# peterhpark/neuroclear

Measured on AMD Instinct MI355X. Metric: voxels/sec, higher is better.
Workload: dtype f32

## Files before the change

### include/nc_hip.h

```cpp
#ifndef NC_HIP_H
#define NC_HIP_H

#include <stddef.h>
#include <stdint.h>

#ifdef __cplusplus
extern "C" {
#endif

#define NC_OK 0
#define NC_ERR_SHAPE (-1)
#define NC_ERR_WS (-2)
#define NC_ERR_HIP (-3)
#define NC_ERR_ARG (-4)

const char* nc_last_error(void);
int nc_version(void);
int nc_conv_fwd_path(int C, int K, int kd, int kh, int kw, int stride, int pad);
int nc_conv_wgrad_path(int C, int K, int kd, int kh, int kw, int stride, int pad);
void nc_prof_begin(double min_flop);
int nc_prof_end(int max, int* cls, double* flop, float* ms);
int nc_prof_end2(int max, int* cls, double* flop, float* ms, double* abytes);
void nc_set_force_direct(int on);
void nc_sconv_set_cfg(int cfg);
// ... 128 lines not shown
int nc_assemble_scatter_add(const float* cube, float* acc, int P0, int P1, int P2, int roi, int overlap, int border,
                            int index, void* stream);
int nc_assemble_finalize(const float* acc, void* out, int out_is_u16, int P0, int P1, int P2, int L0, int L1, int L2,
                         int roi, int overlap, void* stream);
int nc_assemble_finalize_slab(const float* acc_slab, void* out, int out_is_u16, int P0, int P1, int P2, int L0, int L1, int L2, int roi,
                              int overlap, int z0, int nz, int za, void* stream);

int nc_assemble_merge(const float* acc, float* merged, int L0, int L1, int L2, int roi, int overlap, void* stream);
int nc_radix_hist(const float* x, long n, int pass, unsigned prefix, unsigned* hist4096, void* stream);
int nc_assemble_rescale_finalize(const float* merged, void* out, int out_is_u16, int L0, int L1, int L2, int roi,
                                 int overlap, float lo, float hi, float range, void* stream);

size_t nc_match_histograms_ws_bytes(long n);
int nc_match_histograms(const float* source, const float* tmpl, float* out, long n, void* ws, size_t ws_bytes,
                        void* stream);

int nc_spectral_norm_fwd(const float* w_orig, float* u, float* v, float* w_out, float* sigma, float* scratch_k, int K, int M,
                         int power_iteration, float eps, void* stream);
int nc_spectral_norm_bwd(const float* g, const float* w_sn, const float* u, const float* v, const float* sigma, float* dw_orig, int K,
                         int M, void* stream);

size_t nc_patchgan_param_floats(int n_layers, int ndf, int nd);
size_t nc_patchgan_saved_floats(int B, int D, int H, int W, int n_layers, int ndf, int nd);
size_t nc_patchgan_ws_bytes(int B, int D, int H, int W, int n_layers, int ndf, int nd);
int nc_patchgan_out_shape(int B, int D, int H, int W, int n_layers, int ndf, int nd, int* oD, int* oH, int* oW);
int nc_patchgan_fwd(const float* params, const float* x, float* y, float* saved, int B, int D, int H, int W,
                    int n_layers, int ndf, int nd, void* ws, size_t ws_bytes, void* stream);
int nc_patchgan_bwd(const float* params, const float* x, const float* saved, const float* dy, float* dx, float* dparams,
                    int B, int D, int H, int W, int n_layers, int ndf, int nd, void* ws, size_t ws_bytes, void* stream);
int nc_patchgan_fwd_part(const float* params, const float* x, float* y, float* saved, int Btot, int b0, int B, int D, int H,
                         int W, int n_layers, int ndf, int nd, void* ws, size_t ws_bytes, void* stream);
int nc_patchgan_bwd_part(const float* params, const float* x, const float* saved, const float* dy, float* dx, int Btot, int b0,
                         int B, int D, int H, int W, int n_layers, int ndf, int nd, void* ws, size_t ws_bytes, void* stream);
size_t nc_patchgan_gp_saved_floats(int B, int D, int H, int W, int n_layers, int ndf, int nd);
size_t nc_patchgan_gp_ws_bytes(int B, int D, int H, int W, int n_layers, int ndf, int nd);
int nc_patchgan_gp_fwd(const float* params, const float* x, float* g, float* pen, float* saved, int B, int D, int H, int W, int n_layers,
                       int ndf, int nd, float constant, float lambda_gp, void* ws, size_t ws_bytes, void* stream);
int nc_patchgan_gp_bwd(const float* params, const float* x, const float* saved, const float* g, const float* dpen, float* dparams, float* dx,
                       int B, int D, int H, int W, int n_layers, int ndf, int nd, float constant, float lambda_gp, void* ws, size_t ws_bytes,
                       void* stream);

size_t nc_unet_deconv_fwd_ws_bytes(int N, int S0, int S1, int S2);
int nc_unet_deconv_fwd(const float* params, const float* x, float* y, int N, int S0, int S1, int S2, void* ws,
                       size_t ws_bytes, void* stream);


size_t nc_unet_deconv_param_floats(void);
size_t nc_unet_deconv_saved_floats(int N, int S0, int S1, int S2);
size_t nc_unet_deconv_train_ws_bytes(int N, int S0, int S1, int S2);
int nc_unet_deconv_train_fwd(const float* params, const float* x, float* y, float* saved, int N, int S0, int S1, int S2,
                             void* ws, size_t ws_bytes, void* stream, unsigned* kept);
int nc_unet_deconv_bwd(const float* params, const float* x, const float* y, const float* saved, const float* dy, float* dx,
                       float* dparams, int N, int S0, int S1, int S2, void* ws, size_t ws_bytes, void* stream, unsigned kept);
void nc_set_unet_lean(int on);
int nc_get_unet_lean(void);
void nc_set_unet_wprep(int on);
int nc_get_unet_wprep(void);
int nc_set_in_bwd_fold(int on);
int nc_get_in_bwd_fold(void);
int nc_in_bwd_launches(int which, int reset);
int nc_set_stream_passes(int on);
int nc_get_stream_passes(void);
int nc_unet_wprep_layout(int N, int S0, int S1, int S2, int block, int form, size_t* pack_off, size_t* pack_bytes, size_t* cell_off,
                         size_t* bound_off);
int nc_s3x_pack_h2_debug(const float* w, int C, int K, int form, const unsigned* cell_a, const unsigned* cell_b, void* wp, unsigned* wcell,
                         void* stream);
// ... 138 lines not shown
```

### neuroclear_amd/csrc/common.hpp

```cpp
#pragma once
#include <hip/hip_runtime.h>

#include <cstdarg>
#include <cstdio>

#include "../../include/nc_hip.h"
#include "switches.hpp"

namespace nc {

void set_error(const char* fmt, ...);

inline int check_launch(const char* what) {
  hipError_t e = hipGetLastError();
  if (e != hipSuccess) {
    set_error("%s: %s", what, hipGetErrorString(e));
    return NC_ERR_HIP;
  }
  return NC_OK;
}

inline long cdiv(long a, long b) { return (a + b - 1) / b; }

int raise_dyn_lds(const void* kernel, int bytes, const char* who);
// ... 49 lines not shown

int conv_fwd_direct(const float* x, const float* w, const float* b, float* y, const ConvDims& d, hipStream_t s);
int conv_dgrad_direct(const float* dy, const float* w, float* dx, const ConvDims& d, hipStream_t s);
int conv_wgrad_direct(const float* x, const float* dy, float* dw, const ConvDims& d, hipStream_t s);
int bias_grad(const float* dy, float* db, int N, int K, long S, void* ws, size_t wsb, hipStream_t s);
static constexpr size_t kBiasGradWsBytes = 64 * 1024 * sizeof(double);

bool mfma_fwd_supported(const ConvDims& d);
bool c1k3_fwd_supported(const ConvDims& d);
int conv_fwd_c1k3(const float* x, const float* w, const float* bias, float* y, const ConvDims& d, hipStream_t s, float* stats_part = nullptr);
size_t c1k3_stats_bytes(const ConvDims& d);
int c1k3_stats_finalize(const float* stats_part, const float* bias, const ConvDims& d, float eps, float* mean, float* rstd, hipStream_t s);
bool mfma_dgrad_supported(const ConvDims& d);
bool mfma_wgrad_supported(const ConvDims& d);
size_t mfma_ws_bytes(const ConvDims& d);
size_t mfma_fwd_ws_bytes(const ConvDims& d);
int conv_fwd_mfma(const float* x, const float* w, const float* b, float* y, const ConvDims& d, void* ws, size_t wsb,
                  hipStream_t s);
int conv_dgrad_mfma(const float* dy, const float* w, float* dx, const ConvDims& d, void* ws, size_t wsb,
                    hipStream_t s);
int conv_wgrad_mfma(const float* x, const float* dy, float* dw, const ConvDims& d, void* ws, size_t wsb,
                    hipStream_t s);

bool gemm_fwd_supported(const ConvDims& d);
bool gemm_dgrad_supported(const ConvDims& d);
bool gemm_wgrad_supported(const ConvDims& d);
size_t gemm_ws_bytes(const ConvDims& d);
int conv_fwd_gemm(const float* x, const float* w, const float* b, float* y, const ConvDims& d, void* ws, size_t wsb,
                  hipStream_t s);
int conv_dgrad_gemm(const float* dy, const float* w, float* dx, const ConvDims& d, void* ws, size_t wsb,
                    hipStream_t s);
int conv_wgrad_gemm(const float* x, const float* dy, float* dw, const ConvDims& d, void* ws, size_t wsb,
                    hipStream_t s);

bool sconv_fwd_supported(const ConvDims& d);
bool sconv_dgrad_supported(const ConvDims& d);
size_t sconv_ws_bytes(const ConvDims& d);
bool p2d_fwd_supported(const ConvDims& d);
bool p2d_dgrad_supported(const ConvDims& d);
size_t p2d_ws_bytes(const ConvDims& d);
int conv_fwd_p2d(const float* x, const float* w, const float* bias, float* y, const ConvDims& d, void* ws, size_t wsb, hipStream_t s);
int conv_dgrad_p2d(const float* dy, const float* w, float* dx, const ConvDims& d, void* ws, size_t wsb, hipStream_t s);
bool p2d_wgrad_supported(const ConvDims& d);
size_t p2d_wgrad_ws_bytes(const ConvDims& d);
int conv_wgrad_p2d(const float* x, const float* dy, float* dw, const ConvDims& d, void* ws, size_t wsb, hipStream_t s);
int conv_fwd_sconv(const float* x, const float* w, const float* bias, float* y, const ConvDims& d, void* ws, size_t wsb, hipStream_t s);
int conv_dgrad_sconv(const float* dy, const float* w, float* dx, const ConvDims& d, void* ws, size_t wsb, hipStream_t s);
int conv2d_k3_num_cfgs();
bool conv2d_k3_fwd_supported(const ConvDims& d);
bool conv2d_k3_dgrad_supported(const ConvDims& d);
size_t conv2d_k3_ws_bytes(const ConvDims& d);
int conv_fwd_k3(const float* x, const float* w, const float* bias, float* y, const ConvDims& d, void* ws, size_t wsb, hipStream_t s);
int conv_dgrad_k3(const float* dy, const float* w, float* dx, const ConvDims& d, void* ws, size_t wsb, hipStream_t s);
bool conv2d_k3_reflect_ok(const ConvDims& d);
int conv_fwd_k3_reflect(const float* x, const float* w, const float* bias, float* y, const ConvDims& d, void* ws, size_t wsb, hipStream_t s);
int conv_dgrad_k3_reflect_ext(const float* dy, const float* w, float* dxe, const ConvDims& d, void* ws, size_t wsb, hipStream_t s);
int reflect_pad_fwd(const float* x, float* y, long NC, int H, int W, int p, hipStream_t s);
int reflect_pad_bwd(const float* g, float* dx, long NC, int H, int W, int p, hipStream_t s);
bool sconv_wgrad_supported(const ConvDims& d);
size_t sconv_wgrad_ws_bytes(const ConvDims& d);
int conv_wgrad_sconv(const float* x, const float* dy, float* dw, const ConvDims& d, void* ws, size_t wsb, hipStream_t s);

bool pg1_supported(const ConvDims& d);
size_t pg1_ws_bytes(const ConvDims& d);
int conv_fwd_pg1(const float* x, const float* w, const float* bias, float* y, const ConvDims& d, float slope, hipStream_t s);
int conv_wgrad_pg1(const float* x, const float* g, const float* act, float slope, float* dw, float* db, const ConvDims& d,
// ... 239 lines not shown
```

### neuroclear_amd/csrc/misc.hip

```cpp
#include "common.hpp"

namespace nc {

__device__ __forceinline__ void plane_dims(int D, int H, int W, int axis, int& A, int& B) {
  A = axis == 0 ? H : D;
  B = axis == 2 ? H : W;
}
__device__ __forceinline__ long vol_index(int D, int H, int W, int axis, int a, int b, int s) {
  if (axis == 0) return ((long)s * H + a) * W + b;
  if (axis == 1) return ((long)a * H + s) * W + b;
  return ((long)a * H + b) * W + s;
}

__global__ void k_slice_bwd(const float* __restrict__ dout, float* __restrict__ dvol, int NC, int D, int H, int W,
                            int axis, int index) {
  int A, B;
  plane_dims(D, H, W, axis, A, B);
  const long S = (long)D * H * W, total = (long)NC * S;
  for (long i = (long)blockIdx.x * blockDim.x + threadIdx.x; i < total; i += (long)gridDim.x * blockDim.x) {
    const long nc = i / S, r = i % S;
    const int x = (int)(r % W), y = (int)((r / W) % H), z = (int)(r / ((long)W * H));
    const int s = axis == 0 ? z : axis == 1 ? y : x;
    const int a = axis == 0 ? y : z;
    const int b = axis == 2 ? y : x;
// ... 96 lines not shown
}
__global__ void k_l1_bwd(const float* __restrict__ a, const float* __restrict__ b, long n,
                         const float* __restrict__ gscale, float* __restrict__ da) {
  const float g = gscale[0] / (float)n;
  for (long i = (long)blockIdx.x * blockDim.x + threadIdx.x; i < n; i += (long)gridDim.x * blockDim.x) {
    const float d = a[i] - b[i];
    da[i] = d > 0.f ? g : d < 0.f ? -g : 0.f;
  }
}

__global__ void k_adam(float* __restrict__ p, const float* __restrict__ g, float* __restrict__ m,
                       float* __restrict__ v, long n, float b1, float b2, float eps, float step_size,
                       float bc2_sqrt) {
  for (long i = (long)blockIdx.x * blockDim.x + threadIdx.x; i < n; i += (long)gridDim.x * blockDim.x) {
    const float gi = g[i];
    const float wl = 1.f - b1;
    const float mi = wl < 0.5f ? m[i] + wl * (gi - m[i]) : gi - (gi - m[i]) * (1.f - wl);
    const float vi = v[i] * b2 + gi * gi * (1.f - b2);
    m[i] = mi;
    v[i] = vi;
    const float denom = sqrtf(vi) / bc2_sqrt + eps;
    p[i] = p[i] - step_size * (mi / denom);
  }
}

static unsigned flat_grid(long n) {
  long b = cdiv(n, 256);
  if (b > 8192) b = 8192;
  if (b < 1) b = 1;
  return (unsigned)b;
}
static constexpr int kLossBlocks = 256;

}

using namespace nc;

extern "C" {

static int vol_check(const char* what, int NC, int D, int H, int W, int axis) {
  if (NC < 1 || D < 1 || H < 1 || W < 1 || axis < 0 || axis > 2) {
    set_error("%s: bad shape/axis", what);
    return NC_ERR_SHAPE;
  }
  return NC_OK;
}
static int axis_len(int D, int H, int W, int axis) { return axis == 0 ? D : axis == 1 ? H : W; }

int nc_slice_fwd(const float* vol, float* out, int NC, int D, int H, int W, int axis, int index, void* stream) {
  if (!vol || !out) { set_error("slice_fwd: null pointer"); return NC_ERR_ARG; }
  if (int e = vol_check("slice_fwd", NC, D, H, W, axis)) return e;
  if (index < 0 || index >= axis_len(D, H, W, axis)) { set_error("slice_fwd: index out of range"); return NC_ERR_SHAPE; }
  hipLaunchKernelGGL(k_mip_fwd, dim3(flat_grid((long)NC * D * H * W / axis_len(D, H, W, axis))), dim3(256), 0,
                     (hipStream_t)stream, vol, out, (int32_t*)nullptr, NC, D, H, W, axis, index, 1);
  return check_launch("slice_fwd");
}
int nc_slice_bwd(const float* dout, float* dvol, int NC, int D, int H, int W, int axis, int index, void* stream) {
  if (!dout || !dvol) { set_error("slice_bwd: null pointer"); return NC_ERR_ARG; }
  if (int e = vol_check("slice_bwd", NC, D, H, W, axis)) return e;
  if (index < 0 || index >= axis_len(D, H, W, axis)) { set_error("slice_bwd: index out of range"); return NC_ERR_SHAPE; }
  hipLaunchKernelGGL(k_slice_bwd, dim3(flat_grid((long)NC * D * H * W)), dim3(256), 0, (hipStream_t)stream, dout, dvol,
                     NC, D, H, W, axis, index);
  return check_launch("slice_bwd");
}
int nc_mip_fwd(const float* vol, float* out, int32_t* arg, int NC, int D, int H, int W, int axis, int start, int depth,
               void* stream) {
// ... 92 lines not shown
```

### neuroclear_amd/csrc/nets.hip

```cpp
#include "common.hpp"
#include "patchgan_plan.hpp"

using namespace nc;

namespace {

size_t align256(size_t b) { return (b + 255) & ~(size_t)255; }

}

#define NC_TRY(expr) do { int e_ = (expr); if (e_) return e_; } while (0)

extern "C" {

size_t nc_patchgan_param_floats(int n_layers, int ndf, int nd) {
  PgPlan P;
  return pg_plan(P, 1, nd == 3 ? 64 : 1, 64, 64, n_layers, ndf, nd) ? P.params : 0;
}

size_t nc_patchgan_saved_floats(int B, int D, int H, int W, int n_layers, int ndf, int nd) {
  PgPlan P;
  return pg_plan(P, B, D, H, W, n_layers, ndf, nd) ? P.saved : 0;
}

// ... 107 lines not shown
        NC_TRY(nc_instnorm_act_bwd_dbias(gin, praw, mean, rstd, 0.2f, graw, dparams + pl.b_off, B, pl.K, S, iws, P.in_ws,
                                         stream));
        have_db = true;
      } else {
        NC_TRY(nc_instnorm_act_bwd(gin, praw, mean, rstd, 0.2f, graw, B * pl.K, S, iws, P.in_ws, stream));
      }
    } else if (i == 1 && P.fused0) {
      graw = gin;
    } else {
      NC_TRY(nc_leaky_relu_bwd(gin, praw, 0.2f, graw, (long)B * pl.K * S, stream));
    }
    g = graw;
  }
  return NC_OK;
}

int nc_patchgan_bwd(const float* params, const float* x, const float* saved, const float* dy, float* dx, float* dparams,
                    int B, int D, int H, int W, int n_layers, int ndf, int nd, void* ws, size_t ws_bytes, void* stream) {
  if (!params || !x || !saved || !dy) { set_error("patchgan_bwd: null pointer"); return NC_ERR_ARG; }
  PgPlan P;
  if (!pg_plan(P, B, D, H, W, n_layers, ndf, nd)) { set_error("patchgan_bwd: bad shape"); return NC_ERR_SHAPE; }
  if (!ws || ws_bytes < nc_patchgan_ws_bytes(B, D, H, W, n_layers, ndf, nd)) { set_error("patchgan_bwd: workspace too small"); return NC_ERR_WS; }
  return pg_bwd(P, params, x, saved, dy, dx, dparams, B, 0, B, nd, ws, stream);
}

int nc_patchgan_bwd_part(const float* params, const float* x, const float* saved, const float* dy, float* dx, int Btot, int b0,
                         int B, int D, int H, int W, int n_layers, int ndf, int nd, void* ws, size_t ws_bytes, void* stream) {
  if (!params || !x || !saved || !dy || !dx) { set_error("patchgan_bwd_part: null pointer"); return NC_ERR_ARG; }
  PgPlan P;
  if (B < 1 || b0 < 0 || b0 + B > Btot || !pg_plan(P, Btot, D, H, W, n_layers, ndf, nd)) { set_error("patchgan_bwd_part: bad shape"); return NC_ERR_SHAPE; }
  if (!ws || ws_bytes < nc_patchgan_ws_bytes(Btot, D, H, W, n_layers, ndf, nd)) { set_error("patchgan_bwd_part: workspace too small"); return NC_ERR_WS; }
  return pg_bwd(P, params, x, saved, dy, dx, nullptr, Btot, b0, B, nd, ws, stream);
}
}
```

### neuroclear_amd/models/axial_to_lateral_gan_apollo_model.py

```python
import itertools
import os

import numpy as np
import torch

from .. import ops
from . import networks
from .base_model import BaseModel


class FlatAdam(torch.optim.Optimizer):

    def __init__(self, params, lr, betas, eps=1e-8, overlap_all_reduce=False):
        params = list(params)
        super().__init__(params, dict(lr=lr, betas=betas, eps=eps))
        self.params = params
        dev = params[0].device
        n = sum(p.numel() for p in params)
        self.flat = torch.empty(n, dtype=torch.float32, device=dev)
        self.grad = torch.zeros(n, dtype=torch.float32, device=dev)
        self.exp_avg = torch.zeros(n, dtype=torch.float32, device=dev)
        self.exp_avg_sq = torch.zeros(n, dtype=torch.float32, device=dev)
        off = 0
        for p in params:
# ... 77 lines not shown
                else:
                    dist.all_reduce(self.grad[b['lo']:b['hi']])
                b['work'], b['seen'] = None, 0
        else:
            dist.all_reduce(self.grad)
        self.grad.div_(ws)

    @torch.no_grad()
    def step(self, closure=None):
        self._collect()
        self.state_step += 1
        g = self.param_groups[0]
        ops.adam_step(self.flat, self.grad, self.exp_avg, self.exp_avg_sq, g['lr'], g['betas'][0], g['betas'][1],
                      g['eps'], self.state_step)
        ops.bump_param_generation(self.flat)


class AxialToLateralGANApolloModel(BaseModel):
    @staticmethod
    def modify_commandline_options(parser, is_train=True):
        parser.set_defaults(no_dropout=True)
        if is_train:
            parser.add_argument('--lambda_A', type=float, default=10.0, help='weight for cycle loss (A -> B -> A)')
            parser.add_argument('--gan_mode', type=str, default='vanilla', help='[vanilla| lsgan | wgangp]')
            parser.add_argument('--lambda_plane', type=int, nargs='+', default=[1, 1, 1])
            parser.add_argument('--randomize_projection_depth', action='store_true')
            parser.add_argument('--projection_depth', type=int, default=10)
            parser.add_argument('--min_projection_depth', type=int, default=2)
        parser.add_argument('--netG_B', type=str, default='deep_linear_gen')
        return parser

    _d_streams_on = os.environ.get('NC_D_STREAMS', '1') != '0'
    _d_on_main = os.environ.get('NC_D_MAIN', '1') != '0'
    _d_nstreams = int(os.environ.get('NC_D_NSTREAMS', '4'))

    def __init__(self, opt):
        BaseModel.__init__(self, opt)
        self._d_streams = []
        self._fwd_done = None
        self.loss_names = ['D_A_lateral', 'D_A_axial', 'G_A', 'G_A_lateral', 'G_A_axial', 'cycle',
                           'D_B_lateral', 'D_B_axial', 'G_B', 'G_B_lateral', 'G_B_axial']
        self.gan_mode = opt.gan_mode
        self.gen_dimension, self.dis_dimension = 3, 2
        self.randomize_projection_depth = opt.randomize_projection_depth
        if not self.randomize_projection_depth:
            self.projection_depth_custom = opt.projection_depth
        else:
            self.max_projection_depth = opt.projection_depth
            self.min_projection_depth = opt.min_projection_depth
        self.visual_names = ['real', 'fake', 'rec'] * 2
        tot = float(opt.lambda_plane[0] + opt.lambda_plane[1] + opt.lambda_plane[2])
        self.lambda_plane_target, self.lambda_slice, self.lambda_proj = [f / tot for f in opt.lambda_plane]
        self.lateral_axis, self.axial_1_axis, self.axial_2_axis = 0, 1, 2
        self.model_names = ['G_A', 'G_B', 'D_A_lateral', 'D_A_axial', 'D_B_lateral', 'D_B_axial'] if self.isTrain \
            else ['G_A', 'G_B']
        G = networks.define_G
        self.netG_A = G(opt.input_nc, opt.output_nc, opt.ngf, opt.netG, opt.norm, not opt.no_dropout, opt.init_type,
                        opt.init_gain, self.gpu_ids, dimension=self.gen_dimension)
        self.netG_B = G(opt.output_nc, opt.input_nc, opt.ngf, opt.netG_B, opt.norm, not opt.no_dropout, opt.init_type,
                        opt.init_gain, self.gpu_ids, dimension=self.gen_dimension)
        if self.isTrain:
            def D(nc):
                return networks.define_D(nc, opt.ndf, opt.netD, opt.n_layers_D, opt.norm, opt.init_type,
                                         opt.init_gain, False, self.gpu_ids, dimension=self.dis_dimension)
            self.netD_A_axial = D(opt.output_nc)
            self.netD_A_lateral = D(opt.output_nc)
# ... 19 lines not shown
        self.cube_shape = self.real.shape
        self.num_slice = self.cube_shape[-3]
        if not self.randomize_projection_depth:
            self.projection_depth = self.projection_depth_custom
        else:
            self.projection_depth = np.random.randint(max(2, self.min_projection_depth),
                                                      self.max_projection_depth + 1)

    _early_DA = os.environ.get('NC_D_EARLY', '0') != '0'

    def forward(self):
        self.fake = self.netG_A(self.real)
        self._fake_done = None
        if self.real.is_cuda and self._d_streams_on and self._early_DA and self.isTrain:
            self._fake_done = torch.cuda.Event()
            self._fake_done.record()
        self.rec = self.netG_B(self.fake)

    def _slice(self, input, slice_axis):
        return ops.volume_slice(input, slice_axis, np.random.randint(input.shape[-1]))

    def _proj(self, input, slice_axis):
        start = np.random.randint(0, input.shape[-1] - self.projection_depth)
        return ops.volume_mip(input, slice_axis, start, self.projection_depth)

    @staticmethod
    def _D(netD, planes):
        if getattr(netD, 'one_plane_per_call', False):
            return [netD(pl) for pl in planes]
        pred = netD(planes[0] if len(planes) == 1 else torch.cat(planes, 0))
        n = planes[0].shape[0]
        return [pred[i * n:(i + 1) * n] for i in range(len(planes))]

    def _D_many(self, jobs, loss_fn, after=None, backward=False):
        def run(i, net, planes_fn):
            res = loss_fn(i, self._D(net, planes_fn()))
            if backward:
                tot = res if torch.is_tensor(res) else sum(res[1:], res[0])
                tot.backward()
            return res
        if not self._d_streams_on or not self.real.is_cuda:
            return [run(i, net, fn) for i, (net, fn) in enumerate(jobs)]
        main = torch.cuda.current_stream()
        on_main = self._d_on_main and len(jobs) > 3 and not backward
        nside = len(jobs) - 1 if on_main else len(jobs)
        ns = min(nside, self._d_nstreams)
        while len(self._d_streams) < ns:
            self._d_streams.append(torch.cuda.Stream(device=self.device))
        out = []
        for i, (net, fn) in enumerate(jobs[:nside]):
            st = self._d_streams[i % ns]
            ev = after[i] if isinstance(after, (list, tuple)) else after
            if ev is not None:
                st.wait_event(ev)
            else:
                st.wait_stream(main)
            with torch.cuda.stream(st):
                out.append(run(i, net, fn))
        if on_main:
            out.append(run(nside, *jobs[nside]))
        for i in range(ns):
            main.wait_stream(self._d_streams[i])
        return out

    def iter_f(self, input, function, slice_axis):
        return function(self._slice(input, slice_axis))

    def proj_f(self, input, function, slice_axis):
        return function(self._proj(input, slice_axis))
# ... 25 lines not shown
        self.loss_D_A_axial_1 = self._d_loss(p[0], p[1])
        self.loss_D_A_axial_2 = self._d_loss(p[2], p[3])
        (self.loss_D_A_axial_1 + self.loss_D_A_axial_2).backward()
        self.loss_D_A_axial = (self.loss_D_A_axial_1 + self.loss_D_A_axial_2) * 0.5

    def backward_D_B_lateral(self):
        self.loss_D_B_lateral = self.backward_D_slice(self.netD_B_lateral, self.real, self.rec, self.lateral_axis,
                                                      self.lateral_axis)

    def backward_D_B_axial(self):
        rd = self.rec.detach()
        planes = [self._slice(self.real, self.axial_1_axis), self._slice(rd, self.axial_1_axis),
                  self._slice(self.real, self.axial_2_axis), self._slice(rd, self.axial_2_axis)]
        p = self._D(self.netD_B_axial, planes)
        self.loss_D_B_axial_1 = self._d_loss(p[0], p[1])
        self.loss_D_B_axial_2 = self._d_loss(p[2], p[3])
        (self.loss_D_B_axial_1 + self.loss_D_B_axial_2).backward()
        self.loss_D_B_axial = (self.loss_D_B_axial_1 + self.loss_D_B_axial_2) * 0.5

    def backward_G(self):
        lambda_A = self.opt.lambda_A
        g = self.criterionGAN
        f, r = self.fake, self.rec
        la, a1, a2 = self.lateral_axis, self.axial_1_axis, self.axial_2_axis
        jobs = [(self.netD_A_lateral, lambda: [self._proj(f, la)]),
                (self.netD_A_axial, lambda: [self._proj(f, a1), self._proj(f, a2)]),
                (self.netD_B_lateral, lambda: [self._slice(r, la)]),
                (self.netD_B_axial, lambda: [self._slice(r, a1), self._slice(r, a2)])]

        def loss(i, p):
            if i % 2 == 0:
                return g(p[0], True) * self.lambda_plane_target
            return g(p[0], True) * self.lambda_slice + g(p[1], True) * self.lambda_slice
        fd = getattr(self, '_fake_done', None)
        (self.loss_G_A_lateral, self.loss_G_A_axial, self.loss_G_B_lateral, self.loss_G_B_axial) = \
            self._D_many(jobs, loss, after=[fd, fd, None, None] if fd is not None else None)
        self.loss_G_A = self.loss_G_A_lateral + self.loss_G_A_axial * 0.5
        self.loss_G_B = self.loss_G_B_lateral + self.loss_G_B_axial * 0.5
        self.loss_cycle = self.criterionCycle(self.rec, self.real) * lambda_A
        self.loss_G = self.loss_G_A + self.loss_G_B + self.loss_cycle
        self.loss_G.backward()

    def backward_D_all(self):
        fd, rd = self.fake.detach(), self.rec.detach()
        real = self.real
        la, a1, a2 = self.lateral_axis, self.axial_1_axis, self.axial_2_axis
        sl, pj = self._slice, self._proj
        jobs = [(self.netD_A_lateral, lambda: [sl(real, la), pj(fd, la)]),
                (self.netD_A_axial, lambda: [sl(real, la), pj(fd, a1), sl(real, la), pj(fd, a2)]),
                (self.netD_B_lateral, lambda: [sl(real, la), sl(rd, la)]),
                (self.netD_B_axial, lambda: [sl(real, a1), sl(rd, a1), sl(real, a2), sl(rd, a2)])]

        def loss(i, p):
            if i % 2 == 0:
                return (self._d_loss(p[0], p[1]),)
            return (self._d_loss(p[0], p[1]), self._d_loss(p[2], p[3]))
        (l_al,), (l_a1, l_a2), (l_bl,), (l_b1, l_b2) = self._D_many(jobs, loss, after=self._fwd_done, backward=True)
        self.loss_D_A_lateral = l_al
        self.loss_D_A_axial_1, self.loss_D_A_axial_2 = l_a1, l_a2
        self.loss_D_A_axial = (l_a1 + l_a2) * 0.5
        self.loss_D_B_lateral = l_bl
        self.loss_D_B_axial_1, self.loss_D_B_axial_2 = l_b1, l_b2
        self.loss_D_B_axial = (l_b1 + l_b2) * 0.5

    def optimize_parameters(self):
        Ds = [self.netD_A_lateral, self.netD_A_axial, self.netD_B_lateral, self.netD_B_axial]
        self.forward()
        self._fwd_done = None
        if self.real.is_cuda and self._d_streams_on:
# ... 14 lines not shown
```

### neuroclear_amd/models/networks.py

```python
import functools
import os

import torch
import torch.nn as nn
from torch.nn import init
from torch.optim import lr_scheduler

from .. import ops
from .._lib import P, check, lib


class Identity(nn.Module):
    def forward(self, x):
        return x


class InstanceNormAct(nn.Module):

    def __init__(self, num_features, slope=0.0, eps=1e-5):
        super().__init__()
        self.num_features, self.slope, self.eps = num_features, slope, eps

    def forward(self, x, link=None, nxt=None):
        return ops.instance_norm_act(x, self.slope, self.eps, link, nxt)
# ... 539 lines not shown
        seq = [Conv(input_nc, ndf, kw, 2, padw, dimension=dimension), LeakyReLU(0.2)]
        nf_mult = 1
        for n in range(1, n_layers):
            nf_prev, nf_mult = nf_mult, min(2 ** n, 8)
            seq += [Conv(ndf * nf_prev, ndf * nf_mult, kw, 2, padw, bias=use_bias, dimension=dimension)]
            seq += [norm_layer(ndf * nf_mult, 0.2), FusedActivation()] if norm_layer else [Identity(), LeakyReLU(0.2)]
        nf_prev, nf_mult = nf_mult, min(2 ** n_layers, 8)
        seq += [Conv(ndf * nf_prev, ndf * nf_mult, kw, 1, padw, bias=use_bias, dimension=dimension)]
        seq += [norm_layer(ndf * nf_mult, 0.2), FusedActivation()] if norm_layer else [Identity(), LeakyReLU(0.2)]
        seq += [Conv(ndf * nf_mult, 1, kw, 1, padw, dimension=dimension)]
        self.model = nn.Sequential(*seq)
        self._cfg = (n_layers, ndf, dimension)
        self._fusable = _is_instance_norm(norm_layer) and input_nc == 1 and 1 <= n_layers <= 6

    def _fused_on(self, input):
        return self._fusable and input.is_cuda and os.environ.get('NC_FUSED_PATCHGAN', '1') != '0'

    def forward(self, input):
        if self._fused_on(input):
            return ops.patchgan(input, list(self.parameters()), *self._cfg)
        return _run_linked(self.model, input)

    def can_share(self, input):
        return self._fused_on(input) and not any(p.requires_grad for p in self.parameters())

    def forward_fake_half(self, input, share, src, axis):
        return ops.patchgan_fake_half(input, list(self.parameters()), *self._cfg, share, src=src, axis=axis)

    def share_matches(self, share, fake, axis):
        return share is not None and share.matches(list(self.parameters()), self._cfg, fake, axis)

    def forward_join_real(self, input, share):
        return ops.patchgan_join_real(input, list(self.parameters()), *self._cfg, share)


class KernelPatchDiscriminator(nn.Module):

    def __init__(self, input_nc, ndf=64, n_layers=5, norm_layer=None, dimension=3):
        super().__init__()
        use_bias = _is_instance_norm(norm_layer)
        self.dimension, self.instance = dimension, use_bias
        self.batch = norm_layer is not None and not use_bias
        self.first_layer = Conv(input_nc, ndf, 7, 1, 0, bias=use_bias, dimension=dimension)
        seq = []
        for _ in range(1, n_layers - 1):
            seq += [Conv(ndf, ndf, 1, 1, 0, bias=use_bias, dimension=dimension)]
            seq += [norm_layer(ndf, 0.0), FusedActivation()] if norm_layer else [Identity(), LeakyReLU(0.0)]
        self.feature_block = nn.Sequential(*seq)
        self.final_layer = Conv(ndf, 1, 1, 1, 0, bias=use_bias, dimension=dimension)
        self._ndf = ndf
        self._fusable = use_bias and input_nc == 1 and ndf == 64 and n_layers == 5

    def _fused_on(self, input):
        return self._fusable and input.is_cuda and os.environ.get('NC_FUSED_KGAN', '1') != '0'

    def _check(self, input):
        nd = self.dimension
        sp = tuple(input.shape[2:])
        if len(sp) != nd or min(sp) < 7:
            raise ValueError('KernelPatchDiscriminator: input %s: every one of the %d spatial edges must be at least 7 '
                             '(first_layer is a 7^%d conv with padding 0)' % (tuple(input.shape), nd, nd))
        if self.instance:
            ops.kgan_dims(input.shape, nd)
        elif self.batch and self.training:
            n = input.shape[0]
            for e in sp:
# ... 67 lines not shown
        net = NLayerDiscriminator(input_nc, ndf, n_layers_D, norm_layer, use_sigmoid, dimension)
    elif netD == 'pixel':
        net = PixelDiscriminator(input_nc, ndf, norm_layer, dimension)
    elif netD == 'basic_SN':
        net = NLayerDiscriminatorSN(input_nc, ndf, 3, norm_layer, use_sigmoid, dimension)
    elif netD == 'n_layers_SN':
        net = NLayerDiscriminatorSN(input_nc, ndf, n_layers_D, norm_layer, use_sigmoid, dimension)
    elif netD == 'kernelGAN':
        net = KernelPatchDiscriminator(input_nc, ndf, 5, norm_layer, dimension)
    else:
        raise NotImplementedError('Discriminator model name [%s] is not recognized' % netD)
    return init_net(net, init_type, init_gain, gpu_ids)


class GANLoss(nn.Module):

    def __init__(self, gan_mode, target_real_label=1.0, target_fake_label=0.0):
        super().__init__()
        self.register_buffer('real_label', torch.tensor(target_real_label))
        self.register_buffer('fake_label', torch.tensor(target_fake_label))
        self.gan_mode = gan_mode
        self._real, self._fake = float(target_real_label), float(target_fake_label)
        if gan_mode not in ('lsgan', 'vanilla') and 'wgan' not in gan_mode:
            raise NotImplementedError('gan mode %s not implemented' % gan_mode)

    def __call__(self, prediction, target_is_real):
        if self.gan_mode == 'lsgan':
            return ops.mse_const(prediction, self._real if target_is_real else self._fake)
        if self.gan_mode == 'vanilla':
            return ops.bce_logits_const(prediction, self._real if target_is_real else self._fake)
        m = ops.mean(prediction)
        return -m if target_is_real else m


def _gp_unsupported(netD, xs):
    name = type(netD).__name__
    if not isinstance(netD, NLayerDiscriminator):
        return '%s (only the PatchGAN NLayerDiscriminator, --netD basic | n_layers, has one)' % name
    if not netD._fusable:
        return '%s without instance norm or with input_nc != 1 (the fused path covers --norm instance, one input channel)' % name
    if netD._cfg[2] != 2:
        return '%s with dimension=%d (the penalty covers the 2-D discriminators)' % (name, netD._cfg[2])
    for x in xs:
        if not x.is_cuda:
            return '%s on a %s input (there is no CPU path)' % (name, x.device.type)
    if not netD._fused_on(xs[0]):
        return '%s with NC_FUSED_PATCHGAN=0 (the penalty runs only on the fused path)' % name
    return None


def cal_gradient_penalty(netD, real_data, fake_data, device, type='mixed', constant=1.0, lambda_gp=10.0):
    if lambda_gp > 0.0:
        if type not in ('real', 'fake', 'mixed'):
            raise NotImplementedError('{} not implemented'.format(type))
        why = _gp_unsupported(netD, {'real': [real_data], 'fake': [fake_data], 'mixed': [real_data, fake_data]}[type])
        if why is not None:
            raise NotImplementedError('cal_gradient_penalty: no HIP path for %s' % why)
        if type == 'real':
            interpolatesv = real_data
        elif type == 'fake':
            interpolatesv = fake_data
        else:
            alpha = torch.rand(real_data.shape[0], 1, device=device)
            alpha = alpha.expand(real_data.shape[0], real_data.nelement() // real_data.shape[0]).contiguous().view(*real_data.shape)
            interpolatesv = alpha * real_data + ((1 - alpha) * fake_data)
        interpolatesv.requires_grad_(True)
# ... 6 lines not shown
```

### neuroclear_amd/ops.py

```python
import ctypes
import os

import torch

from . import _lib
from ._lib import I, P, check, lib

_ws_cache = {}

prof = None


def prof_start(min_flop=0.0):
    global prof
    prof = []
    lib().nc_prof_begin(min_flop)


_PATH = {0: 'direct', 1: 'mfma', 2: 'gemm', 3: 'flat', 4: 'taps', 5: 'k1', 6: 'to1', 7: 'img', 8: 'pg1', 9: 'split', 10: 'split2d', 11: 'split',
         12: 'lk'}


def prof_stop():
    global prof
# ... 1073 lines not shown
        ws = _net_ws(ctx, x.device)
        check(L.nc_patchgan_fwd_part(_ptr(packed), _ptr(share.x), _ptr(share.y), _ptr(share.saved), 2 * B, 0, B, *dims[1:], _ptr(ws),
                                     ws.numel(), _stream()), 'nc_patchgan_fwd_part')
        ctx.save_for_backward(share.x, share.saved)
        y = share.y
        share.release()
        return y

    @staticmethod
    def backward(ctx, dy):
        x, saved = ctx.saved_tensors
        dy = dy.contiguous()
        dx = torch.empty_like(x) if ctx.needs_input_grad[0] else None
        dpar, ws = _net_backward(ctx, x.device, 'fused PatchGAN: the parameters were updated between this forward and its backward')
        check(lib().nc_patchgan_bwd(_ptr(ctx.packed), _ptr(x), _ptr(saved), _ptr(dy), _ptr(dx), _ptr(dpar), *ctx.net[2], _ptr(ws),
                                    ws.numel(), _stream()), 'nc_patchgan_bwd')
        return _net_grads(ctx, dx[:x.shape[0] // 2] if dx is not None else None, dpar)


def patchgan_fake_half(x, params, n_layers, ndf, dimension, share, src=None, axis=None):
    y = _PatchGANFakeHalf.apply(x, (int(n_layers), int(ndf), int(dimension)), share, *params)
    share.src, share.src_version, share.axis = src, (src._version if src is not None else None), axis
    return y


def patchgan_join_real(x, params, n_layers, ndf, dimension, share):
    return _PatchGANJoinReal.apply(x, (int(n_layers), int(ndf), int(dimension)), share, *params)


def patchgan(x, params, n_layers, ndf, dimension):
    return _PatchGAN.apply(x, (int(n_layers), int(ndf), int(dimension)), *params)


class _PatchGANGP(torch.autograd.Function):

    @staticmethod
    def forward(ctx, x, cfg, *params):
        n_layers, ndf, nd, constant, lambda_gp = cfg
        x = x.contiguous()

        def dims():
            if nd != 2 or x.dim() != 4 or x.shape[1] != 1:
                raise _lib.NcError('patchgan_gp: the fused penalty covers 2-D inputs [B, 1, H, W], got %s (nd=%d)' % (tuple(x.shape), nd))
            return (x.shape[0], 1, x.shape[2], x.shape[3], n_layers, ndf, nd)

        L = lib()
        packed, dims = _net_forward(ctx, x, params, first=2, dims=dims, ws_bytes=L.nc_patchgan_gp_ws_bytes, tag='patchgan',
                                    n_params=L.nc_patchgan_param_floats(n_layers, ndf, nd), count_msg=_PG_COUNT % (n_layers, ndf))
        nsaved = L.nc_patchgan_gp_saved_floats(*dims)
        if nsaved == 0:
            raise _lib.NcError('patchgan_gp: shape %s not covered (n_layers=%d)' % (tuple(x.shape), n_layers))
        saved = torch.empty(nsaved, dtype=torch.float32, device=x.device)
        g = torch.empty_like(x)
        pen = torch.empty((), dtype=torch.float32, device=x.device)
        ws = _net_ws(ctx, x.device)
        check(L.nc_patchgan_gp_fwd(_ptr(packed), _ptr(x), _ptr(g), _ptr(pen), _ptr(saved), *dims, constant, lambda_gp, _ptr(ws),
                                   ws.numel(), _stream()), 'nc_patchgan_gp_fwd')
        ctx.mark_non_differentiable(g)
        ctx.save_for_backward(x, saved, g)
        ctx.gp = (constant, lambda_gp)
        return pen, g

    @staticmethod
    def backward(ctx, dpen, dg):
        x, saved, g = ctx.saved_tensors
        dpen = dpen.to(torch.float32).contiguous()
# ... 462 lines not shown
```

Baseline: 55.97 million.

## Fuse frozen PatchGAN forward, generator loss and input-gradient into one call

Adds a fused generator-loss path for a frozen PatchGAN discriminator. One native call runs the forward pass, computes per-plane lsgan/vanilla/wgan losses and the loss gradient in a single kernel, then runs the backward pass to dx. The loss value is returned as a tensor whose autograd backward only scales the precomputed dx. This removes separate autograd graph construction, loss kernels and the later discriminator backward dispatch. In exchange it adds workspace, and dx is computed eagerly inside forward.

```diff
diff --git a/include/nc_hip.h b/include/nc_hip.h
--- a/include/nc_hip.h
+++ b/include/nc_hip.h
@@ -184,6 +184,9 @@
                          int W, int n_layers, int ndf, int nd, void* ws, size_t ws_bytes, void* stream);
 int nc_patchgan_bwd_part(const float* params, const float* x, const float* saved, const float* dy, float* dx, int Btot, int b0,
                          int B, int D, int H, int W, int n_layers, int ndf, int nd, void* ws, size_t ws_bytes, void* stream);
+size_t nc_patchgan_gloss_ws_bytes(int B, int D, int H, int W, int n_layers, int ndf, int nd, int planes);
+int nc_patchgan_gloss(const float* params, const float* x, int B, int D, int H, int W, int n_layers, int ndf, int nd, int planes, int mode,
+                      float target, const float* weights, float* losses, float* dx, void* ws, size_t ws_bytes, void* stream);
 size_t nc_patchgan_gp_saved_floats(int B, int D, int H, int W, int n_layers, int ndf, int nd);
 size_t nc_patchgan_gp_ws_bytes(int B, int D, int H, int W, int n_layers, int ndf, int nd);
 int nc_patchgan_gp_fwd(const float* params, const float* x, float* g, float* pen, float* saved, int B, int D, int H, int W, int n_layers,
diff --git a/neuroclear_amd/csrc/common.hpp b/neuroclear_amd/csrc/common.hpp
--- a/neuroclear_amd/csrc/common.hpp
+++ b/neuroclear_amd/csrc/common.hpp
@@ -105,6 +105,11 @@
                     hipStream_t s);
 int conv_wgrad_gemm(const float* x, const float* dy, float* dw, const ConvDims& d, void* ws, size_t wsb,
                     hipStream_t s);
+
+constexpr int kGlossMaxPlanes = 16;
+size_t gloss_loss_ws_bytes(int planes);
+int gloss_loss_dy(const float* pred, int planes, long n, int mode, float target, const float* weights, float* losses, float* dy, void* ws,
+                  hipStream_t s);
 
 bool sconv_fwd_supported(const ConvDims& d);
 bool sconv_dgrad_supported(const ConvDims& d);
diff --git a/neuroclear_amd/csrc/misc.hip b/neuroclear_amd/csrc/misc.hip
--- a/neuroclear_amd/csrc/misc.hip
+++ b/neuroclear_amd/csrc/misc.hip
@@ -152,6 +152,58 @@
 }
 static constexpr int kLossBlocks = 256;
 
+struct GlossWeights { float w[kGlossMaxPlanes]; };
+__global__ __launch_bounds__(256) void k_gloss_partial(const float* __restrict__ pred, float target, int mode, long n, GlossWeights gw,
+                                                       double* __restrict__ part, float* __restrict__ dy) {
+  const float* a = pred + (long)blockIdx.y * n;
+  double acc = 0.0;
+  for (long i = (long)blockIdx.x * 256 + threadIdx.x; i < n; i += (long)gridDim.x * 256) {
+    if (mode >= 2) {
+      const float x = a[i];
+      acc += mode == 3 ? (double)x : (double)(fmaxf(x, 0.f) - x * target + log1pf(expf(-fabsf(x))));
+      continue;
+    }
+    const float d = a[i] - target;
+    acc += (double)d * (double)d;
+  }
+  __shared__ double red[4];
+  for (int o = 32; o > 0; o >>= 1) acc += __shfl_down(acc, o);
+  if ((threadIdx.x & 63) == 0) red[threadIdx.x >> 6] = acc;
+  __syncthreads();
+  if (threadIdx.x == 0) part[(size_t)blockIdx.y * gridDim.x + blockIdx.x] = (red[0] + red[1]) + (red[2] + red[3]);
+  if (!dy) return;
+  float* dp = dy + (long)blockIdx.y * n;
+  if (mode == 0) {
+    const float g = gw.w[blockIdx.y] * (2.0f / (float)n);
+    for (long i = (long)blockIdx.x * 256 + threadIdx.x; i < n; i += (long)gridDim.x * 256) dp[i] = (a[i] - target) * g;
+  } else {
+    const float g = gw.w[blockIdx.y] / (float)n;
+    for (long i = (long)blockIdx.x * 256 + threadIdx.x; i < n; i += (long)gridDim.x * 256)
+      dp[i] = mode == 3 ? g : (1.f / (1.f + expf(-a[i])) - target) * g;
+  }
+}
+__global__ void k_gloss_final(const double* __restrict__ part, int nb, long n, GlossWeights gw, int planes, float* __restrict__ out) {
+  const int p = threadIdx.x;
+  if (blockIdx.x == 0 && p < planes) {
+    double s = 0.0;
+    for (int i = 0; i < nb; ++i) s += part[(size_t)p * nb + i];
+    out[p] = (float)(s / (double)n) * gw.w[p];
+  }
+}
+
+size_t gloss_loss_ws_bytes(int planes) { return (size_t)planes * kLossBlocks * sizeof(double); }
+
+int gloss_loss_dy(const float* pred, int planes, long n, int mode, float target, const float* weights, float* losses, float* dy, void* ws,
+                  hipStream_t s) {
+  GlossWeights gw{};
+  for (int p = 0; p < planes; ++p) gw.w[p] = weights[p];
+  long nb = cdiv(n, 1024);
+  if (nb > kLossBlocks) nb = kLossBlocks;
+  hipLaunchKernelGGL(k_gloss_partial, dim3((unsigned)nb, (unsigned)planes), dim3(256), 0, s, pred, target, mode, n, gw, (double*)ws, dy);
+  hipLaunchKernelGGL(k_gloss_final, dim3(1), dim3(64), 0, s, (const double*)ws, (int)nb, n, gw, planes, losses);
+  return check_launch("patchgan_gloss loss");
+}
+
 }
 
 using namespace nc;
diff --git a/neuroclear_amd/csrc/nets.hip b/neuroclear_amd/csrc/nets.hip
--- a/neuroclear_amd/csrc/nets.hip
+++ b/neuroclear_amd/csrc/nets.hip
@@ -163,4 +163,46 @@
   if (!ws || ws_bytes < nc_patchgan_ws_bytes(Btot, D, H, W, n_layers, ndf, nd)) { set_error("patchgan_bwd_part: workspace too small"); return NC_ERR_WS; }
   return pg_bwd(P, params, x, saved, dy, dx, nullptr, Btot, b0, B, nd, ws, stream);
 }
-}
+
+namespace {
+struct GlossLayout { size_t saved, y, dy, part, total; long npred; };
+bool gloss_layout(PgPlan& P, GlossLayout& G, int B, int D, int H, int W, int n_layers, int ndf, int nd, int planes) {
+  if (planes < 1 || planes > kGlossMaxPlanes || B < 1 || B % planes || !pg_plan(P, B, D, H, W, n_layers, ndf, nd)) return false;
+  G.npred = (long)B * P.oD * P.oH * P.oW;
+  size_t o = align256(nc_patchgan_ws_bytes(B, D, H, W, n_layers, ndf, nd));
+  G.saved = o; o += align256(P.saved * sizeof(float));
+  G.y = o; o += align256((size_t)G.npred * sizeof(float));
+  G.dy = o; o += align256((size_t)G.npred * sizeof(float));
+  G.part = o; o += align256(gloss_loss_ws_bytes(planes));
+  G.total = o;
+  return true;
+}
+}
+
+size_t nc_patchgan_gloss_ws_bytes(int B, int D, int H, int W, int n_layers, int ndf, int nd, int planes) {
+  PgPlan P;
+  GlossLayout G;
+  return gloss_layout(P, G, B, D, H, W, n_layers, ndf, nd, planes) ? G.total : 0;
+}
+
+int nc_patchgan_gloss(const float* params, const float* x, int B, int D, int H, int W, int n_layers, int ndf, int nd, int planes, int mode,
+                      float target, const float* weights, float* losses, float* dx, void* ws, size_t ws_bytes, void* stream) {
+  if (!params || !x || !weights || !losses) { set_error("patchgan_gloss: null pointer"); return NC_ERR_ARG; }
+  if (mode != 0 && mode != 2 && mode != 3) { set_error("patchgan_gloss: mode %d (0 lsgan, 2 vanilla, 3 wgan)", mode); return NC_ERR_ARG; }
+  PgPlan P;
+  GlossLayout G;
+  if (!gloss_layout(P, G, B, D, H, W, n_layers, ndf, nd, planes)) {
+    set_error("patchgan_gloss: bad shape (B=%d must hold 1 .. %d planes of equal size, got planes=%d)", B, kGlossMaxPlanes, planes);
+    return NC_ERR_SHAPE;
+  }
+  if (!ws || ws_bytes < G.total) { set_error("patchgan_gloss: workspace too small"); return NC_ERR_WS; }
+  char* wb = (char*)ws;
+  float* saved = (float*)(wb + G.saved);
+  float* y = (float*)(wb + G.y);
+  float* dy = dx ? (float*)(wb + G.dy) : nullptr;
+  NC_TRY(pg_fwd(P, params, x, y, saved, B, 0, B, nd, ws, stream));
+  NC_TRY(gloss_loss_dy(y, planes, G.npred / planes, mode, target, weights, losses, dy, wb + G.part, (hipStream_t)stream));
+  if (!dx) return NC_OK;
+  return pg_bwd(P, params, x, saved, dy, dx, nullptr, B, 0, B, nd, ws, stream);
+}
+}
diff --git a/neuroclear_amd/models/axial_to_lateral_gan_apollo_model.py b/neuroclear_amd/models/axial_to_lateral_gan_apollo_model.py
--- a/neuroclear_amd/models/axial_to_lateral_gan_apollo_model.py
+++ b/neuroclear_amd/models/axial_to_lateral_gan_apollo_model.py
@@ -133,6 +133,7 @@
 
     _d_streams_on = os.environ.get('NC_D_STREAMS', '1') != '0'
     _d_on_main = os.environ.get('NC_D_MAIN', '1') != '0'
+    _d_gloss = os.environ.get('NC_D_GLOSS', '1') != '0'
     _d_nstreams = int(os.environ.get('NC_D_NSTREAMS', '4'))
 
     def __init__(self, opt):
@@ -218,9 +219,12 @@
         n = planes[0].shape[0]
         return [pred[i * n:(i + 1) * n] for i in range(len(planes))]
 
-    def _D_many(self, jobs, loss_fn, after=None, backward=False):
+    def _D_many(self, jobs, loss_fn, after=None, backward=False, whole=None):
         def run(i, net, planes_fn):
-            res = loss_fn(i, self._D(net, planes_fn()))
+            planes = planes_fn()
+            res = whole(i, net, planes) if whole is not None else None
+            if res is None:
+                res = loss_fn(i, self._D(net, planes))
             if backward:
                 tot = res if torch.is_tensor(res) else sum(res[1:], res[0])
                 tot.backward()
@@ -312,9 +316,16 @@
             if i % 2 == 0:
                 return g(p[0], True) * self.lambda_plane_target
             return g(p[0], True) * self.lambda_slice + g(p[1], True) * self.lambda_slice
+
+        def gloss(i, net, planes):
+            if not (self._d_gloss and hasattr(net, 'can_gloss') and net.can_gloss(planes[0])):
+                return None
+            w = self.lambda_plane_target if i % 2 == 0 else self.lambda_slice
+            ls = net.gloss(planes, g, True, [w] * len(planes))
+            return ls[0] if i % 2 == 0 else ls[0] + ls[1]
         fd = getattr(self, '_fake_done', None)
         (self.loss_G_A_lateral, self.loss_G_A_axial, self.loss_G_B_lateral, self.loss_G_B_axial) = \
-            self._D_many(jobs, loss, after=[fd, fd, None, None] if fd is not None else None)
+            self._D_many(jobs, loss, after=[fd, fd, None, None] if fd is not None else None, whole=gloss)
         self.loss_G_A = self.loss_G_A_lateral + self.loss_G_A_axial * 0.5
         self.loss_G_B = self.loss_G_B_lateral + self.loss_G_B_axial * 0.5
         self.loss_cycle = self.criterionCycle(self.rec, self.real) * lambda_A
diff --git a/neuroclear_amd/models/networks.py b/neuroclear_amd/models/networks.py
--- a/neuroclear_amd/models/networks.py
+++ b/neuroclear_amd/models/networks.py
@@ -595,6 +595,13 @@
 
     def forward_join_real(self, input, share):
         return ops.patchgan_join_real(input, list(self.parameters()), *self._cfg, share)
+
+    def can_gloss(self, input):
+        return self._fused_on(input) and not any(p.requires_grad for p in self.parameters())
+
+    def gloss(self, planes, criterion, target_is_real, weights):
+        mode, target, sign = criterion.gloss_args(target_is_real)
+        return ops.patchgan_gloss(planes, list(self.parameters()), self._cfg, mode, target, [sign * w for w in weights])
 
 
 class KernelPatchDiscriminator(nn.Module):
@@ -728,6 +735,11 @@
         m = ops.mean(prediction)
         return -m if target_is_real else m
 
+    def gloss_args(self, target_is_real):
+        if self.gan_mode in ('lsgan', 'vanilla'):
+            return self.gan_mode, (self._real if target_is_real else self._fake), 1.0
+        return 'wgan', 0.0, (-1.0 if target_is_real else 1.0)
+
 
 def _gp_unsupported(netD, xs):
     name = type(netD).__name__
diff --git a/neuroclear_amd/ops.py b/neuroclear_amd/ops.py
--- a/neuroclear_amd/ops.py
+++ b/neuroclear_amd/ops.py
@@ -1129,6 +1129,45 @@
     return _PatchGAN.apply(x, (int(n_layers), int(ndf), int(dimension)), *params)
 
 
+GLOSS_MODES = {'lsgan': 0, 'vanilla': 2, 'wgan': 3}
+
+
+class _PatchGANGloss(torch.autograd.Function):
+    @staticmethod
+    def forward(ctx, x, cfg, gl, *params):
+        n_layers, ndf, nd = cfg
+        planes, mode, target, weights = gl
+        if any(ctx.needs_input_grad[3:]):
+            raise _lib.NcError('patchgan_gloss: the discriminator must be frozen (generator loss)')
+        x = x.contiguous()
+        L = lib()
+        packed, dims = _net_forward(ctx, x, params, first=3, dims=lambda: _pg_dims(x, cfg, x.shape[0]), ws_bytes=L.nc_patchgan_ws_bytes,
+                                    tag='patchgan', n_params=L.nc_patchgan_param_floats(*cfg), count_msg=_PG_COUNT % (n_layers, ndf))
+        if planes < 1 or x.shape[0] % planes or len(weights) != planes:
+            raise _lib.NcError('patchgan_gloss: %d planes and %d weights for a batch of %d' % (planes, len(weights), x.shape[0]))
+        losses = torch.empty(planes, dtype=torch.float32, device=x.device)
+        dx = torch.empty_like(x) if ctx.needs_input_grad[0] else None
+        B, D, H, W = dims[:4]
+        ws = workspace(L.nc_patchgan_gloss_ws_bytes(B, D, H, W, n_layers, ndf, nd, planes), x.device, 'patchgan_gloss')
+        w = (ctypes.c_float * planes)(*weights)
+        check(L.nc_patchgan_gloss(_ptr(packed), _ptr(x), B, D, H, W, n_layers, ndf, nd, planes, mode, target, w, _ptr(losses), _ptr(dx),
+                                  _ptr(ws), ws.numel(), _stream()), 'nc_patchgan_gloss')
+        ctx.dx, ctx.planes = dx, planes
+        return losses
+
+    @staticmethod
+    def backward(ctx, g):
+        dx = ctx.dx
+        gx = (dx.view(ctx.planes, -1) * g.reshape(ctx.planes, 1)).view(dx.shape) if dx is not None else None
+        return (gx, None, None) + (None,) * len(ctx.shapes)
+
+
+def patchgan_gloss(planes, params, cfg, mode, target, weights):
+    x = planes[0] if len(planes) == 1 else torch.cat(list(planes), 0)
+    gl = (len(planes), GLOSS_MODES[mode], float(target), tuple(float(w) for w in weights))
+    return _PatchGANGloss.apply(x, tuple(int(c) for c in cfg), gl, *params)
+
+
 class _PatchGANGP(torch.autograd.Function):
 
     @staticmethod
```

Result: no change. 56.44 million, median of 6 (+0.8%).
